# jorr3/Alphazero-4-player-chess

Measured on AMD Instinct MI355X. Metric: MCTS simulations/sec (whole node), 256 games×400 sims, 10-block ResNet, higher is better.
Workload: dtype fp16

## Files before the change

### alphazero-4-player-chess_amd/csrc/fpc_nn.h

```cpp
#pragma once
#include <hip/hip_runtime.h>

#include <algorithm>
#include <cstdlib>
#include <cstring>
#include <string>
#include <vector>

#include "fpc_tree_kernels.h"
#include "fpc_pack.h"
#include "fpc_tower.h"
#include "fpc_towerw.h"

namespace fpc {

typedef __attribute__((ext_vector_type(8))) __bf16 bf16x8_t;
typedef __attribute__((ext_vector_type(8))) _Float16 f16x8_t;
typedef __attribute__((ext_vector_type(16))) float f32x16_t;
typedef __attribute__((ext_vector_type(4))) uint32_t u32x4_t;
typedef __attribute__((ext_vector_type(2))) uint32_t u32x2_t;
typedef __attribute__((ext_vector_type(4))) float f32x4_t;

template <int DT>
struct E16;
// ... 334 lines not shown
  hipStream_t stream = nullptr;
  std::vector<void *> allocs;
  uint16_t *in16 = nullptr;
  uint16_t *act[3] = {nullptr, nullptr, nullptr};
  uint16_t *yv = nullptr;
  uint16_t *xfc = nullptr;
  float *d_logits = nullptr;
  float *d_stats = nullptr;
  float *d_value = nullptr;
  ConvW stem, pconv, vconv;
  std::vector<ConvW> c1, c2;
  uint16_t *fcw = nullptr;
  float *fcb = nullptr, *vw = nullptr;
  float *fc_part = nullptr;
  int fc_G1 = 0, fc_s1 = FC_SPLITK, fc_s2 = FC_SPLITK;
  int fc_layout = 1;
  int fc_gw = 256;
  unsigned char *towerW = nullptr;
  unsigned char *stemW = nullptr;
  float *towerB = nullptr;
  bool use_tower = false;
  int tower_waves = 8;
  bool tower_compact = true;
  bool tower_taploop = true;
  int towerw_rows = 1;
  bool use_towerw = false;
  void (*mark_fn)(void *, int) = nullptr;
  void *mark_ctx = nullptr;
  float vb = 0.f;
  bool attr_conv[2][3] = {{false, false, false}, {false, false, false}}, attr_tower[2] = {false, false}, attr_towerw[2] = {false, false}, attr_fc[2] = {false, false}, attr_gemv = false;

  template <class T>
  int dmalloc(T **p, size_t count, std::string *err) {
    void *q = nullptr;
    if (hipMalloc(&q, count * sizeof(T)) != hipSuccess) { *err = "hipMalloc failed in NN (" + std::to_string(count * sizeof(T)) + " bytes)"; return FPC_ENOMEM; }
    (void)hipMemset(q, 0, count * sizeof(T));
    allocs.push_back(q);
    *p = (T *)q;
    return 0;
  }

  int init(const DevCfg &c, int max_games, int nn_dtype, hipStream_t s, std::string *) {
    dc = c; Gmax = max_games; dtype = nn_dtype ? 1 : 0; stream = s;
    P = c.R + 2; PP = P * P;
    Mrows = ((max_games * PP + CONV_BM - 1) / CONV_BM) * CONV_BM;
    Gpad = ((max_games + 255) / 256) * 256;
// ... 77 lines not shown
    c1.assign(nblocks, ConvW()); c2.assign(nblocks, ConvW());
    for (int i = 0; i < nblocks; ++i) { if ((rc = conv(c1[i], F, Fp)) || (rc = conv(c2[i], F, Fp))) return rc; }
    if ((rc = conv(pconv, F, 128))) return rc;
    if ((rc = conv(vconv, F, 128))) return rc;
    if ((rc = dmalloc(&fcw, (size_t)Np * Kp, err)) || (rc = dmalloc(&fcb, (size_t)Np, err))) return rc;
    if ((rc = dmalloc(&vw, (size_t)dc.RR * 32, err))) return rc;
    const size_t rows = (size_t)Mrows + 2 * guard;
    if ((rc = dmalloc(&in16, rows * 32, err))) return rc;
    for (auto &a : act) if ((rc = dmalloc(&a, rows * F, err))) return rc;
    if ((rc = dmalloc(&yv, rows * 32, err))) return rc;
    if ((rc = dmalloc(&xfc, (size_t)Gpad * Kp, err))) return rc;
    if ((rc = dmalloc(&fc_part, (size_t)2 * FC_SPLITK * Gpad * Np, err))) return rc;
    plan_fc();
    if ((rc = dmalloc(&d_logits, (size_t)Gmax * dc.A, err))) return rc;
    if ((rc = dmalloc(&d_stats, (size_t)Gmax * SM_MAXCH * SM_REC, err))) return rc;
    if ((rc = dmalloc(&d_value, (size_t)Gmax, err))) return rc;
    use_tower = use_towerw = false;
    const bool dev = getenv("FPC_DEV_KNOBS") && atoi(getenv("FPC_DEV_KNOBS")) != 0;
    auto knob = [dev](const char *name, int dflt) { const char *v = dev ? getenv(name) : nullptr; return v ? atoi(v) : dflt; };
    const bool no_tower = knob("FPC_NO_TOWER", 0) != 0;
    tower_waves = knob("FPC_TOWER_WAVES", 8);
    tower_compact = knob("FPC_TOWER_COMPACT", 1) != 0;
    tower_taploop = knob("FPC_TOWER_TAPLOOP", 1) != 0;
    if (F == 256 && !no_tower) {
      use_towerw = true;
      towerw_rows = knob("FPC_TOWERW_ROWS", 1);
    } else if (F == 128 && !no_tower) {
      const int kw = knob("FPC_TOWERW", -1);
      use_towerw = kw < 0 ? dc.R != 14 : kw != 0;
      use_tower = !use_towerw;
    }
    const int layers = 2 * nblocks + 2;
    if (use_towerw) {
      const int slab = tww_slab(F), ksn = F / 32;
      if ((rc = dmalloc(&towerW, ((size_t)layers * 9 * ksn + TWW_PAD_SLABS) * slab, err)) || (rc = dmalloc(&stemW, (size_t)9 * slab, err)) ||
          (rc = dmalloc(&towerB, (size_t)layers * 256, err))) return rc;
    } else if (use_tower) {
      if ((rc = dmalloc(&towerW, (size_t)(layers * 9 + 3) * TW_TAP, err)) || (rc = dmalloc(&stemW, (size_t)9 * TW_STEM_TAP, err)) ||
          (rc = dmalloc(&towerB, (size_t)layers * 256, err))) return rc;
    }
    return 0;
  }
  std::vector<ConvW *> convs_in_blob_order() {
    std::vector<ConvW *> v{&stem};
    for (int i = 0; i < nblocks; ++i) { v.push_back(&c1[i]); v.push_back(&c2[i]); }
    v.push_back(&pconv); v.push_back(&vconv);
// ... 103 lines not shown
      in_boards = nullptr;
      t.in16 = in16 + (size_t)guard * 32; t.Wstem = stemW; t.bstem = stem.b; t.Wt = towerW; t.bt = towerB;
      t.xfc = xfc; t.vw = vw; t.value = value_out; t.vb = vb;
      t.L = 2 * nblocks; t.P = P; t.R = dc.R; t.PP = PP; t.NR = PP - P; t.T0 = (P + 1) / 16; t.n_games = n; t.Kp = Kp; t.A_ch = dc.A_ch; t.rules = dc.rules;
#if defined(TW_STAMPS) || defined(TWW_STAMPS)
      static unsigned long long *d_stamps = nullptr;
      if (!d_stamps) { (void)hipMalloc(&d_stamps, 2 * 8 * 16 * 8); }
      (void)hipMemsetAsync(d_stamps, 0, 2 * 8 * 16 * 8, stream);
      t.stamps = d_stamps;
#endif
      const int mt = dc.R <= 8 ? 3 : dc.R <= 11 ? 5 : 7;
      bool &attr = attr_tower[DT];
      if (!attr) {
        (void)hipFuncSetAttribute(reinterpret_cast<const void *>(&k_tower<DT, 3, false, 4>), hipFuncAttributeMaxDynamicSharedMemorySize, TW_LDS);
        (void)hipFuncSetAttribute(reinterpret_cast<const void *>(&k_tower<DT, 5, false, 4>), hipFuncAttributeMaxDynamicSharedMemorySize, TW_LDS);
        (void)hipFuncSetAttribute(reinterpret_cast<const void *>(&k_tower<DT, 7, false, 4>), hipFuncAttributeMaxDynamicSharedMemorySize, TW_LDS);
        (void)hipFuncSetAttribute(reinterpret_cast<const void *>(&k_tower<DT, 7, true, 4>), hipFuncAttributeMaxDynamicSharedMemorySize, TW_LDS);
        (void)hipFuncSetAttribute(reinterpret_cast<const void *>(&k_tower<DT, 7, true, 8>), hipFuncAttributeMaxDynamicSharedMemorySize, TW_LDS);
        (void)hipFuncSetAttribute(reinterpret_cast<const void *>(&k_tower<DT, 3, false, 8>), hipFuncAttributeMaxDynamicSharedMemorySize, TW_LDS);
        (void)hipFuncSetAttribute(reinterpret_cast<const void *>(&k_tower<DT, 5, false, 8>), hipFuncAttributeMaxDynamicSharedMemorySize, TW_LDS);
        (void)hipFuncSetAttribute(reinterpret_cast<const void *>(&k_tower<DT, 7, false, 8>), hipFuncAttributeMaxDynamicSharedMemorySize, TW_LDS);
        (void)hipFuncSetAttribute(reinterpret_cast<const void *>(&k_towerc<DT, false>), hipFuncAttributeMaxDynamicSharedMemorySize, TW_LDS);
        (void)hipFuncSetAttribute(reinterpret_cast<const void *>(&k_towerc<DT, true>), hipFuncAttributeMaxDynamicSharedMemorySize, TW_LDS);
        attr = true;
      }
      if (use_towerw) {
        bool &aw = attr_towerw[DT];
        if (!aw) {
#define FPC_TWW_ATTR(F_, MT_) (void)hipFuncSetAttribute(reinterpret_cast<const void *>(&k_towerw<DT, F_, MT_>), hipFuncAttributeMaxDynamicSharedMemorySize, tww_lds(F_))
#define FPC_TWW_ATTRS(F_) FPC_TWW_ATTR(F_, 2); FPC_TWW_ATTR(F_, 3); FPC_TWW_ATTR(F_, 4); FPC_TWW_ATTR(F_, 5); FPC_TWW_ATTR(F_, 6); FPC_TWW_ATTR(F_, 7)
          FPC_TWW_ATTRS(256); FPC_TWW_ATTRS(128);
#define FPC_TWW_ATTR1(F_, MT_) (void)hipFuncSetAttribute(reinterpret_cast<const void *>(&k_towerw<DT, F_, MT_, true>), hipFuncAttributeMaxDynamicSharedMemorySize, tww_lds(F_))
          FPC_TWW_ATTR1(128, 4); FPC_TWW_ATTR1(256, 4); FPC_TWW_ATTR1(256, 6); FPC_TWW_ATTR1(256, 7); FPC_TWW_ATTR1(256, 8);
          FPC_TWW_ATTR1(256, 9); FPC_TWW_ATTR1(256, 11); FPC_TWW_ATTR1(256, 13);
#undef FPC_TWW_ATTR1
          aw = true;
        }
        const int mtw = tww_mt(dc.R);
        if (mtw < 2 || mtw > 7) { *err = "k_towerw: board size outside 8..14"; return FPC_EINVAL; }
#define FPC_TWW_GO(F_, MT_) hipLaunchKernelGGL((k_towerw<DT, F_, MT_>), dim3(n), dim3(TWW_THREADS), tww_lds(F_), stream, t)
#define FPC_TWW_GOS(F_) switch (mtw) { case 2: FPC_TWW_GO(F_, 2); break; case 3: FPC_TWW_GO(F_, 3); break; case 4: FPC_TWW_GO(F_, 4); break; \
                                       case 5: FPC_TWW_GO(F_, 5); break; case 6: FPC_TWW_GO(F_, 6); break; default: FPC_TWW_GO(F_, 7); break; }
        const int tiles = tww_tiles(dc.R);
        const bool onerow = tiles <= 4 || (F == 256 && towerw_rows != 2);
#define FPC_TWW_GO1(F_, MT_) hipLaunchKernelGGL((k_towerw<DT, F_, MT_, true>), dim3(n), dim3(TWW_THREADS), tww_lds(F_), stream, t)
        if (onerow && F == 128) FPC_TWW_GO1(128, 4);
        else if (onerow) {
          switch (tiles) {
            case 4: FPC_TWW_GO1(256, 4); break;   case 6: FPC_TWW_GO1(256, 6); break;   case 7: FPC_TWW_GO1(256, 7); break;
            case 8: FPC_TWW_GO1(256, 8); break;   case 9: FPC_TWW_GO1(256, 9); break;   case 11: FPC_TWW_GO1(256, 11); break;
            default: FPC_TWW_GO1(256, 13); break;
          }
        } else if (F == 256) { FPC_TWW_GOS(256) } else { FPC_TWW_GOS(128) }
#undef FPC_TWW_GO1
#undef FPC_TWW_GOS
#undef FPC_TWW_GO
      } else if (mt == 3 && tower_waves == 8) hipLaunchKernelGGL((k_tower<DT, 3, false, 8>), dim3(n), dim3(512), TW_LDS, stream, t);
      else if (mt == 3) hipLaunchKernelGGL((k_tower<DT, 3, false, 4>), dim3(n), dim3(256), TW_LDS, stream, t);
      else if (mt == 5 && tower_waves == 8) hipLaunchKernelGGL((k_tower<DT, 5, false, 8>), dim3(n), dim3(512), TW_LDS, stream, t);
      else if (mt == 5) hipLaunchKernelGGL((k_tower<DT, 5, false, 4>), dim3(n), dim3(256), TW_LDS, stream, t);
      else if (P != 16 && tower_waves == 8) hipLaunchKernelGGL((k_tower<DT, 7, false, 8>), dim3(n), dim3(512), TW_LDS, stream, t);
      else if (P != 16) hipLaunchKernelGGL((k_tower<DT, 7, false, 4>), dim3(n), dim3(256), TW_LDS, stream, t);
      else if (tower_waves == 8 && tower_compact && dc.R == 14 && tower_taploop) hipLaunchKernelGGL((k_towerc<DT, true>), dim3(n), dim3(512), TW_LDS, stream, t);
      else if (tower_waves == 8 && tower_compact && dc.R == 14) hipLaunchKernelGGL((k_towerc<DT, false>), dim3(n), dim3(512), TW_LDS, stream, t);
      else if (tower_waves == 8) hipLaunchKernelGGL((k_tower<DT, 7, true, 8>), dim3(n), dim3(512), TW_LDS, stream, t);
      else hipLaunchKernelGGL((k_tower<DT, 7, true, 4>), dim3(n), dim3(256), TW_LDS, stream, t);
      const hipError_t le = hipGetLastError();
      if (le != hipSuccess) { *err = std::string("k_tower launch failed: ") + hipGetErrorString(le); return FPC_ENODEVICE; }
#if defined(TW_STAMPS) || defined(TWW_STAMPS)
      if (getenv("FPC_TW_STAMPS_FILE")) {
        unsigned long long h[2 * 8 * 16];
        (void)hipStreamSynchronize(stream);
        (void)hipMemcpy(h, t.stamps, sizeof(h), hipMemcpyDeviceToHost);
        if (FILE *f = fopen(getenv("FPC_TW_STAMPS_FILE"), "w")) {
          for (int i = 0; i < 2 * 8 * 16; ++i) fprintf(f, "%llu%c", h[i], i % 16 == 15 ? '\n' : ' ');
          fclose(f);
        }
      }
#endif
    } else if ((rc = conv(stem, in16, 32, nullptr, act[0], F, F, 0))) return rc;
    const bool fused = use_tower || use_towerw;
    for (int i = 0; i < nblocks && !fused; ++i) {
      const int t1 = (cur + 1) % 3, t2 = (cur + 2) % 3;
      if ((rc = conv(c1[i], act[cur], F, nullptr, act[t1], F, F, 0))) return rc;
      if ((rc = conv(c2[i], act[t1], F, act[cur], act[t2], F, F, 0))) return rc;
// ... 92 lines not shown
```

### alphazero-4-player-chess_amd/csrc/fpc_tower.h

```cpp
#pragma once
#include <hip/hip_runtime.h>

#include <type_traits>

#include "fpc_tree_kernels.h"

namespace fpc {

typedef __attribute__((ext_vector_type(8))) __bf16 t_bf16x8;
typedef __attribute__((ext_vector_type(8))) _Float16 t_f16x8;
typedef __attribute__((ext_vector_type(4))) float t_f32x4;
typedef __attribute__((ext_vector_type(2))) float t_f32x2;
typedef __attribute__((ext_vector_type(4))) uint32_t t_u32x4;
typedef __attribute__((ext_vector_type(2))) uint32_t t_u32x2;
typedef __attribute__((ext_vector_type(2))) short t_i16x2;

template <int DT>
struct M16;
template <>
struct M16<0> {
  static __device__ __forceinline__ t_f32x4 mfma(t_u32x4 a, t_u32x4 b, t_f32x4 c) {
    return __builtin_amdgcn_mfma_f32_16x16x32_bf16(__builtin_bit_cast(t_bf16x8, a), __builtin_bit_cast(t_bf16x8, b), c, 0, 0, 0);
  }
  static __device__ __forceinline__ uint32_t pack2(float lo, float hi) {
// ... 17 lines not shown
};
__device__ __forceinline__ uint32_t tw_relu2(uint32_t p) {
  return __builtin_bit_cast(uint32_t, __builtin_elementwise_max(__builtin_bit_cast(t_i16x2, p), (t_i16x2{0, 0})));
}

__host__ __device__ constexpr int tw_lay(int CH, int row, int c) {
  return (row >> 3) * (CH * 128) + (c >> 1) * 256 + (c & 1) * 128 + (row & 7) * 16;
}

constexpr int TW_THREADS = 256;
constexpr int TW_BIAS = 0;
constexpr int TW_DUMMY = 2048;
constexpr int TW_VRED = 2560;
constexpr int TW_BOARD = 2624;
constexpr int TW_PACE = 2944;
constexpr int TW_IMG0 = 4096;
constexpr int TW_IMG = 61440;
constexpr int TW_TAP = 32768;
constexpr int TW_RING = TW_IMG0 + TW_IMG;
constexpr int TW_LDS = TW_RING + 3 * TW_TAP;
constexpr int TW_STEM_TAP = 8192;
constexpr int TW_ENC = TW_RING + 9 * TW_STEM_TAP;
static_assert(TW_LDS == 163840, "k_tower uses the whole LDS of a CU");

struct TowerArgs {
  const fpc_board *boards;
  const int *leaf_slot, *leaf_turn;
  int board_stride;
  uint16_t one16;
  const uint16_t *in16;
  const unsigned char *Wstem;
  const float *bstem;
  const unsigned char *Wt;
  const float *bt;
  uint16_t *xfc;
  const float *vw;
  float *value;
  float vb;
  int L, P, R, PP, NR, T0, n_games, Kp, A_ch;
  int rules;
  unsigned long long *stamps;
};

__device__ __forceinline__ void tw_dma_8k(const unsigned char *gsrc_uniform, uint32_t lane_off, uint32_t lds_addr_uniform) {
  uint32_t keep;
  asm volatile(
      "s_mov_b32 %0, m0\n\ts_mov_b32 m0, %3\n\ts_nop 0\n\t"
      "global_load_lds_dwordx4 %1, %2\n\ts_add_u32 m0, m0, 0x400\n\tv_add_u32 %1, 0x400, %1\n\t"
      "global_load_lds_dwordx4 %1, %2\n\ts_add_u32 m0, m0, 0x400\n\tv_add_u32 %1, 0x400, %1\n\t"
      "global_load_lds_dwordx4 %1, %2\n\ts_add_u32 m0, m0, 0x400\n\tv_add_u32 %1, 0x400, %1\n\t"
      "global_load_lds_dwordx4 %1, %2\n\ts_add_u32 m0, m0, 0x400\n\tv_add_u32 %1, 0x400, %1\n\t"
      "global_load_lds_dwordx4 %1, %2\n\ts_add_u32 m0, m0, 0x400\n\tv_add_u32 %1, 0x400, %1\n\t"
      "global_load_lds_dwordx4 %1, %2\n\ts_add_u32 m0, m0, 0x400\n\tv_add_u32 %1, 0x400, %1\n\t"
      "global_load_lds_dwordx4 %1, %2\n\ts_add_u32 m0, m0, 0x400\n\tv_add_u32 %1, 0x400, %1\n\t"
      "global_load_lds_dwordx4 %1, %2\n\t"
      "s_mov_b32 m0, %0"
      : "=&s"(keep), "+v"(lane_off) : "s"(gsrc_uniform), "s"(lds_addr_uniform) : "memory", "scc");
}
__device__ __forceinline__ void tw_dma_4k(const unsigned char *gsrc_uniform, uint32_t lane_off, uint32_t lds_addr_uniform) {
  uint32_t keep;
  asm volatile(
      "s_mov_b32 %0, m0\n\ts_mov_b32 m0, %3\n\ts_nop 0\n\t"
      "global_load_lds_dwordx4 %1, %2\n\ts_add_u32 m0, m0, 0x400\n\tv_add_u32 %1, 0x400, %1\n\t"
      "global_load_lds_dwordx4 %1, %2\n\ts_add_u32 m0, m0, 0x400\n\tv_add_u32 %1, 0x400, %1\n\t"
      "global_load_lds_dwordx4 %1, %2\n\ts_add_u32 m0, m0, 0x400\n\tv_add_u32 %1, 0x400, %1\n\t"
      "global_load_lds_dwordx4 %1, %2\n\t"
      "s_mov_b32 m0, %0"
      : "=&s"(keep), "+v"(lane_off) : "s"(gsrc_uniform), "s"(lds_addr_uniform) : "memory", "scc");
}
template <int OFF>
__device__ __forceinline__ void tw_dma_piece(const unsigned char *gsrc_uniform, uint32_t lane_off) {
  asm volatile("global_load_lds_dwordx4 %0, %1 offset:%2" : : "v"(lane_off), "s"(gsrc_uniform), "i"(OFF) : "memory");
}
__device__ __forceinline__ void tw_set_m0(uint32_t lds_addr_uniform) {
  asm volatile("s_mov_b32 m0, %0\n\ts_nop 0" : : "s"(lds_addr_uniform) : "memory");
}
__device__ __forceinline__ void tw_dma_256(const unsigned char *gsrc_uniform, uint32_t lane_off, uint32_t lds_addr_uniform) {
  uint32_t keep;
  asm volatile("s_mov_b32 %0, m0\n\ts_mov_b32 m0, %3\n\ts_nop 0\n\tglobal_load_lds_dword %1, %2\n\ts_mov_b32 m0, %0"
               : "=&s"(keep) : "v"(lane_off), "s"(gsrc_uniform), "s"(lds_addr_uniform) : "memory");
}

#ifdef TW_STAMPS
#define TW_STAMP(GT, I)                                                                                       \
  do {                                                                                                        \
    if (g.stamps && blockIdx.x == 0 && ((GT) == TW_STAMPS || (GT) == TW_STAMPS + 1)) {                        \
      const unsigned long long t_ = __builtin_amdgcn_s_memtime();                                             \
// ... 3 lines not shown
#else
#define TW_STAMP(GT, I) do {} while (0)
#endif
#ifndef TW_AHEAD
#define TW_AHEAD 2
#endif
#ifndef TW_LOADERS
#define TW_LOADERS 1
#endif
#ifndef TW_STAGGER
#define TW_STAGGER 3
#endif
#ifndef TW_STRIP
#define TW_STRIP 0
#endif
#ifndef TWC_LOADER_TILES
#define TWC_LOADER_TILES 6
#endif

#ifndef TWC_STAGGER
#define TWC_STAGGER 2
#endif

template <int DT, int MT, bool FAST, int NW, int LOAD, bool CMP = false, bool TU = false>
__device__ __forceinline__ void tw_body(const TowerArgs &g) {
  static_assert(!CMP || (!FAST && NW == 8 && TW_LOADERS == 1 && MT == (LOAD == 2 ? TWC_LOADER_TILES : 13 - TWC_LOADER_TILES)), "compact form: 8 waves, 13 row tiles");
  static_assert(!TU || (CMP && TW_STAGGER != 0 && TWC_STAGGER >= 1 && TWC_STAGGER <= 3), "tap-specialised loop: compact form with the burst stream");
  constexpr int CR = 14, CZ = 16;
  constexpr int TB0 = LOAD == 2 ? 0 : TWC_LOADER_TILES;
  constexpr int NT = NW * 64;
  constexpr int WN = NW / 2;
  constexpr int CT = 8 / WN;
  constexpr int PIECES = 4 * LOAD;
  constexpr int DMA_PER_WAVE = PIECES * 1024;
  constexpr int MID = PIECES == 8 ? 4096 : 0;
  constexpr bool STREAM = TW_AHEAD == 2 && !(TW_STAGGER != 0 && NW == 8 && TW_LOADERS == 1);
  constexpr int STAG = (NW == 8 && TW_LOADERS == 1 && LOAD == 0) ? (TU ? TWC_STAGGER : TW_STAGGER) : 0;
  extern __shared__ __attribute__((aligned(16))) unsigned char smem[];
  unsigned char *const img = smem + TW_IMG0;
  unsigned char *const ring = smem + TW_RING;
  const float *const biasbuf = reinterpret_cast<const float *>(smem + TW_BIAS);
  float *const vred = reinterpret_cast<float *>(smem + TW_VRED);
  fpc_board *const lboard = reinterpret_cast<fpc_board *>(smem + TW_BOARD);
  const int tid = threadIdx.x, lane = tid & 63;
  const int wave = __builtin_amdgcn_readfirstlane(tid >> 6);
  const int wm = wave / WN, wn = wave % WN;
  const int li = lane & 15, lq = lane >> 4;
  const int game = blockIdx.x;
  const int P = g.P, NR = g.NR;

  int slot = 0, rot_k = 0;
  if (g.boards) {
    slot = g.leaf_slot[game];
    if (slot < 0) return;
    rot_k = first_leaf_turn(g.leaf_slot, g.leaf_turn, g.n_games);
  }

  const int rbase = CMP ? CZ + TB0 * 16 + li : (g.T0 + wm * MT) * 16 + li;
  uint32_t inmask = 0;
#pragma unroll
  for (int mt = 0; mt < MT; ++mt) {
    const int r = rbase + 16 * mt;
    if (CMP) {
      if (r - CZ < CR * CR) inmask |= 1u << mt;
    } else {
      const int pi = r / P, pj = r - pi * P;
      if (r < g.PP && pi >= 1 && pi <= g.R && pj >= 1 && pj <= g.R) inmask |= 1u << mt;
    }
  }
  auto colmask = [](int mt, int dx) -> uint64_t {
    uint32_t m16 = 0;
    for (int i = 0; i < 16; ++i)
      if (dx != 0 && ((TB0 + mt) * 16 + i) % CR == (dx < 0 ? 0 : CR - 1)) m16 |= 1u << i;
    const uint32_t m32 = m16 * 0x10001u;
    return ((uint64_t)m32 << 32) | m32;
  };
  auto lane_select = [](uint32_t a, uint32_t b, uint64_t m) -> uint32_t {
    uint32_t r;
    asm("v_cndmask_b32_e64 %0, %1, %2, %3" : "=v"(r) : "v"(a), "v"(b), "s"(m));
    return r;
  };
  const int bq = (lq >> 1) * 256 + (lq & 1) * 128;
  const int apart = (li >> 3) * 2048 + (li & 7) * 16 + bq;
  const int apart_s = (li >> 3) * 512 + (li & 7) * 16 + bq;
  const int cb64 = wn * (CT * 16);
  const int cb16 = (wn & 1) * 16;
  const bool vactive = wn < 2;

  for (int c = tid; c < (TW_IMG0 + TW_IMG) / 16; c += NT) reinterpret_cast<t_u32x4 *>(smem)[c] = t_u32x4{0u, 0u, 0u, 0u};
  unsigned char *const enc = smem + TW_ENC;
  const int enc_bytes = CMP ? 240 * 64 : ((NR + 7) >> 3) * 512;
  for (int c = tid; c < enc_bytes / 16; c += NT) reinterpret_cast<t_u32x4 *>(enc)[c] = t_u32x4{0u, 0u, 0u, 0u};
  {
    const t_u32x4 *src = reinterpret_cast<const t_u32x4 *>(g.Wstem);
    t_u32x4 *dst = reinterpret_cast<t_u32x4 *>(ring);
    for (int c = tid; c < 9 * TW_STEM_TAP / 16; c += NT) dst[c] = src[c];
  }
  t_f32x4 bst[CT];
#pragma unroll
  for (int ct = 0; ct < CT; ++ct) bst[ct] = *reinterpret_cast<const t_f32x4 *>(g.bstem + cb64 + ct * 16 + 4 * lq);
  __syncthreads();
  if (g.boards) {
    constexpr int WPB = (int)(sizeof(fpc_board) / 4);
    if (tid < WPB) reinterpret_cast<uint32_t *>(lboard)[tid] =
        reinterpret_cast<const uint32_t *>(g.boards + (size_t)game * g.board_stride + slot)[tid];
    __syncthreads();
    if (g.rules & FPC_RULES_ROTATION) rot_k = lboard->turn;
    for (int r = tid; r < (CMP ? CR * CR : g.PP); r += NT) {
      const int pi = CMP ? r / CR + 1 : r / P, pj = CMP ? r % CR + 1 : r - pi * P;
      if (pi < 1 || pi > g.R || pj < 1 || pj > g.R) continue;
      const uint8_t p = lboard->sq[rot90_src(g.R, rot_k, pi - 1, pj - 1)];
      if (!present(p)) continue;
      const int plane = piece_plane(p, lboard->turn, g.rules);
      *reinterpret_cast<uint16_t *>(enc + tw_lay(4, CMP ? CZ + r : r, plane >> 3) + (plane & 7) * 2) = g.one16;
    }
  } else if (CMP) {
    const uint16_t *src = g.in16 + (size_t)game * g.PP * 32;
    for (int c = tid; c < CR * CR * 4; c += NT) {
      const int q = c >> 2, j = c & 3;
      *reinterpret_cast<t_u32x4 *>(enc + tw_lay(4, CZ + q, j)) =
          *reinterpret_cast<const t_u32x4 *>(src + ((size_t)(q / CR + 1) * P + q % CR + 1) * 32 + j * 8);
    }
  } else {
    const uint16_t *src = g.in16 + (size_t)game * g.PP * 32;
    for (int c = tid; c < NR * 4; c += NT) {
      const int r = c >> 2, j = c & 3;
      *reinterpret_cast<t_u32x4 *>(enc + tw_lay(4, r, j)) = *reinterpret_cast<const t_u32x4 *>(src + (size_t)r * 32 + j * 8);
    }
  }
  __syncthreads();

  t_f32x4 acc[MT][CT];
  t_u32x2 res[MT][CT];

  auto brow = [&](int mt, int shift) -> int {
    int r = rbase + 16 * mt + shift;
    r = r < 0 ? r + NR : r;
    r = r >= NR ? r - NR : r;
    return r;
  };

#pragma unroll
  for (int tap = 0; tap < 9; ++tap) {
    const int shift = (tap / 3 - 1) * (CMP ? CR : P) + (tap % 3 - 1);
    t_u32x4 fa[CT], fb[MT];
#pragma unroll
    for (int ct = 0; ct < CT; ++ct)
      fa[ct] = *reinterpret_cast<const t_u32x4 *>(ring + tap * TW_STEM_TAP + (cb64 + ct * 16) * 64 + apart_s);
#pragma unroll
    for (int mt = 0; mt < MT; ++mt) {
      const int r = CMP ? (int)lane_select((uint32_t)(rbase + 16 * mt + shift), (uint32_t)((rbase + shift) & 7), colmask(mt, tap % 3 - 1)) : brow(mt, shift);
      fb[mt] = *reinterpret_cast<const t_u32x4 *>(enc + (r >> 3) * 512 + (r & 7) * 16 + bq);
    }
#pragma unroll
    for (int mt = 0; mt < MT; ++mt)
#pragma unroll
      for (int ct = 0; ct < CT; ++ct) acc[mt][ct] = M16<DT>::mfma(fa[ct], fb[mt], tap == 0 ? bst[ct] : acc[mt][ct]);
  }
  __syncthreads();

  const int total = (g.L + 2) * 9;
  const uint32_t dma_lane = (uint32_t)lane * 16u;
  const int lw = LOAD == 2 ? (wave & 3) : wave;
  auto issue_bias = [&](int T) {
    if (T % 9 == 0 && T < total && wave < 4) {
      const int l = T / 9;
      tw_dma_256(reinterpret_cast<const unsigned char *>(g.bt + (size_t)l * 256 + wave * 64), (uint32_t)lane * 4u,
                 (uint32_t)__builtin_amdgcn_readfirstlane(TW_BIAS + ((l & 1) * 256 + wave * 64) * 4));
    }
  };
  auto issue_tap = [&](int T) {
    issue_bias(T);
    if (LOAD == 0 || (TW_STRIP & 4)) return;
    const unsigned char *src = g.Wt + (size_t)T * TW_TAP + lw * DMA_PER_WAVE;
    const uint32_t dst = (uint32_t)__builtin_amdgcn_readfirstlane(TW_RING + (T % 3) * TW_TAP + lw * DMA_PER_WAVE);
    if (PIECES == 8) tw_dma_8k(src, dma_lane, dst);
    else tw_dma_4k(src, dma_lane, dst);
  };
  const unsigned char *dsrc = g.Wt;
  auto open_tap = [&](int T) {
    issue_bias(T);
    if (LOAD == 0) return;
    dsrc = g.Wt + (size_t)T * TW_TAP + lw * DMA_PER_WAVE + MID;
    tw_set_m0((uint32_t)__builtin_amdgcn_readfirstlane(TW_RING + (T % 3) * TW_TAP + lw * DMA_PER_WAVE + MID));
  };
  auto piece = [&](auto i_c) {
    constexpr int I = decltype(i_c)::value;
    if (LOAD != 0) tw_dma_piece<I * 1024 - MID>(dsrc, dma_lane);
  };
  issue_tap(0);
  issue_tap(1);
  if (STREAM) {
    open_tap(2);
    piece(std::integral_constant<int, 0>{});
    if (LOAD == 2) piece(std::integral_constant<int, 1>{});
  }

  unsigned char *const dummy = smem + TW_DUMMY + lane * 8;
  unsigned char *const wbase = img + (rbase >> 3) * 2048 + (rbase & 7) * 16 + wn * (CT * 256) + (lane >> 5) * 128 + ((lane >> 4) & 1) * 8;
  auto epilogue = [&](auto res_c) {
    constexpr int RES = decltype(res_c)::value;
    if (TW_STRIP & 16) return;
#pragma unroll
    for (int mt = 0; mt < MT; ++mt) {
      unsigned char *dst = ((inmask >> mt) & 1u) ? wbase + mt * 4096 : dummy;
#pragma unroll
      for (int ct = 0; ct < CT; ++ct) {
        t_f32x4 v = acc[mt][ct];
        if (RES == 2) {
          v[0] += M16<DT>::lo(res[mt][ct][0]); v[1] += M16<DT>::hi(res[mt][ct][0]);
          v[2] += M16<DT>::lo(res[mt][ct][1]); v[3] += M16<DT>::hi(res[mt][ct][1]);
        }
        const t_u32x2 pk = t_u32x2{tw_relu2(M16<DT>::pack2(v[0], v[1])), tw_relu2(M16<DT>::pack2(v[2], v[3]))};
        if (RES != 0) res[mt][ct] = pk;
        *reinterpret_cast<t_u32x2 *>(((inmask >> mt) & 1u) ? dst + ct * 256 : dst) = pk;
      }
      __builtin_amdgcn_sched_barrier(0);
    }
  };
  const std::integral_constant<int, 0> c0{};
  const std::integral_constant<int, 1> c1{};
  const std::integral_constant<int, 2> c2{};
  const std::integral_constant<int, 3> c3{};
  epilogue(c1);
  if (TW_STRIP & 32) { asm volatile("s_waitcnt vmcnt(0)" ::: "memory"); return; }
  if (STREAM) asm volatile("s_waitcnt vmcnt(%0)" ::"n"(PIECES + LOAD) : "memory");
  else asm volatile("s_waitcnt vmcnt(0)" ::: "memory");
  __syncthreads();

  t_u32x4 fa[2][CT], fb[2][MT];
  int gt = 0;
  const unsigned char *wslot;
  const unsigned char *bbase;
  const unsigned char *blast;
  int boff[FAST ? 1 : MT];
  auto set_tap = [&](int tap, int cb) {
    wslot = ring + (gt % 3) * TW_TAP + cb * 256 + apart;
    const int shift = (tap / 3 - 1) * P + (tap % 3 - 1);
    if (FAST) {
      const int r = rbase + shift;
      bbase = img + (r >> 3) * 2048 + (r & 7) * 16 + bq;
      int rl = r + 16 * (MT - 1);
      rl = rl >= NR ? rl - NR : rl;
      blast = img + (rl >> 3) * 2048 + (rl & 7) * 16 + bq;
    } else if (CMP) {
      const int dx = tap % 3 - 1;
      const int r = rbase + (tap / 3 - 1) * CR + dx;
      const uint32_t zoff = (r & 7) * 16 + bq;
      const uint32_t b0 = (r >> 3) * 2048 + zoff;
// ... 16 lines not shown
    asm volatile("" : "+v"(o2));
    wrow = ring + o;
    wrow2 = ring + o2;
  };
  int rrow = rbase - CR;
  auto set_tap_u = [&](auto xn_c) {
    constexpr int XN = decltype(xn_c)::value;
    wslot = XN == 2 ? wrow2 : wrow + XN * TW_TAP;
    const int r = rrow + (XN - 1);
    const uint32_t zoff = (r & 7) * 16 + bq;
    const uint32_t b0 = (r >> 3) * 2048 + zoff;
#pragma unroll
    for (int mt = 0; mt < MT; ++mt)
      boff[mt] = XN == 1 ? (int)(b0 + mt * 4096) : (int)lane_select(b0 + mt * 4096, zoff, colmask(mt, XN - 1));
  };
  auto bptr = [&](int mt) -> const unsigned char * {
    if (FAST) return mt == MT - 1 ? blast : bbase + mt * 4096;
    return img + boff[mt];
  };
  auto kstep = [&](auto mode_c, auto buf_c, auto ksn_c, auto bias_c, const t_f32x4 *b4, auto q_c) {
    constexpr int MODE = decltype(mode_c)::value, B = decltype(buf_c)::value, KSN = decltype(ksn_c)::value;
    constexpr bool BIAS = decltype(bias_c)::value != 0;
    constexpr int N = B ^ 1, Q = decltype(q_c)::value;
    if (!(TW_STRIP & 2)) {
#pragma unroll
      for (int ct = 0; ct < CT; ++ct) fa[N][ct] = *reinterpret_cast<const t_u32x4 *>(wslot + ct * 4096 + KSN * 512);
      fb[N][0] = *reinterpret_cast<const t_u32x4 *>(bptr(0) + KSN * 512);
    }
    __builtin_amdgcn_sched_barrier(0);
#pragma unroll
    for (int mt = 0; mt < MT; ++mt) {
      if (TW_STRIP & 1) {
        if (BIAS) {
#pragma unroll
          for (int ct = 0; ct < (MODE == 0 ? CT : 1); ++ct) acc[mt][ct] = b4[ct];
        }
        asm volatile("" : "+v"(fa[B][0]), "+v"(fb[B][mt]));
      } else if (MODE == 0) {
#pragma unroll
        for (int ct = 0; ct < CT; ++ct) acc[mt][ct] = M16<DT>::mfma(fa[B][ct], fb[B][mt], BIAS ? b4[ct] : acc[mt][ct]);
      } else if (NW == 4 || vactive) {
        acc[mt][0] = M16<DT>::mfma(fa[B][0], fb[B][mt], BIAS ? b4[0] : acc[mt][0]);
      }
      __builtin_amdgcn_sched_barrier(0);
      if (mt + 1 < MT && !(TW_STRIP & 2)) {
        fb[N][mt + 1] = *reinterpret_cast<const t_u32x4 *>(bptr(mt + 1) + KSN * 512);
        __builtin_amdgcn_sched_barrier(0);
      }
      if (STREAM && LOAD != 0) {
        if (mt == (LOAD == 2 ? MT / 3 : MT / 2)) piece(std::integral_constant<int, LOAD * Q>{});
        if (LOAD == 2 && mt == (2 * MT) / 3) piece(std::integral_constant<int, LOAD * Q + 1>{});
        __builtin_amdgcn_sched_barrier(0);
      }
    }
  };
  auto load_b0 = [&]() {
#pragma unroll
    for (int mt = 0; mt < MT; ++mt) fb[0][mt] = *reinterpret_cast<const t_u32x4 *>(bptr(mt));
  };
  const unsigned char *usrc = g.Wt + (size_t)TW_TAP + lw * DMA_PER_WAVE;
  const uint32_t udst = (uint32_t)__builtin_amdgcn_readfirstlane(TW_RING + lw * DMA_PER_WAVE);
  auto tap_u = [&](auto mode_c, auto x_c, const t_f32x4 *b4, const int dy, const int cb_next) {
    constexpr int X = decltype(x_c)::value;
    if (STAG == 2) {
      TW_STAMP(gt, 3);
      __syncthreads();
      TW_STAMP(gt, 4);
    }
    TW_STAMP(gt, 0);
    kstep(mode_c, c1, c2, c0, b4, c2);
    TW_STAMP(gt, 1);
    if (STAG == 1) __syncthreads();
    kstep(mode_c, c0, c3, c0, b4, c3);
    TW_STAMP(gt, 2);
    if (!STAG) {
      asm volatile("s_waitcnt vmcnt(0)" ::: "memory");
      TW_STAMP(gt, 3);
      if (!(TW_STRIP & 8)) __syncthreads();
      TW_STAMP(gt, 4);
      if (LOAD != 0 && !(TW_STRIP & 4)) {
        usrc += TW_TAP;
        tw_dma_8k(usrc, dma_lane, udst + ((X + 2) % 3) * TW_TAP);
      }
      TW_STAMP(gt, 5);
    }
    ++gt;
    if (X == 2) {
      rrow = dy == 1 ? rbase - CR : rrow + CR;
      if (dy == 1) set_wrow(cb_next);
    }
    set_tap_u(std::integral_constant<int, (X + 1) % 3>{});
    TW_STAMP(gt - 1, 6);
    kstep(mode_c, c1, c0, c0, b4, c0);
    TW_STAMP(gt - 1, 7);
  };
  auto run_layer = [&](auto mode_c, const int layer, const int cb, const int cb_next) {
    constexpr int MODE = decltype(mode_c)::value;
    if (TU && wave < 4 && layer + 1 < g.L + 2)
      tw_dma_256(reinterpret_cast<const unsigned char *>(g.bt + (size_t)(layer + 1) * 256 + wave * 64), (uint32_t)lane * 4u,
                 (uint32_t)__builtin_amdgcn_readfirstlane(TW_BIAS + (((layer + 1) & 1) * 256 + wave * 64) * 4));
    t_f32x4 b4[CT];
    {
      const float *bl = biasbuf + (layer & 1) * 256 + cb + 4 * lq;
#pragma unroll
      for (int ct = 0; ct < (MODE == 0 ? CT : 1); ++ct) b4[ct] = *reinterpret_cast<const t_f32x4 *>(bl + ct * 16);
// ... 57 lines not shown
  if (TU) {
    set_wrow(cb64);
    set_tap_u(c0);
  } else {
    set_tap(0, cb64);
  }
#pragma unroll
  for (int ct = 0; ct < CT; ++ct) fa[0][ct] = *reinterpret_cast<const t_u32x4 *>(wslot + ct * 4096);
  load_b0();
  const int nblocks = g.L / 2;
#pragma unroll 1
  for (int blk = 0; blk < nblocks; ++blk) {
    run_layer(c0, 2 * blk, cb64, cb64);
    epilogue(c0);
    __syncthreads();
    load_b0();
    run_layer(c0, 2 * blk + 1, cb64, blk + 1 == nblocks ? cb16 : cb64);
    epilogue(c2);
    __syncthreads();
    load_b0();
  }
  float vpart = 0.f;
  {
    run_layer(c1, g.L, cb16, cb64);
#pragma unroll
    for (int mt = 0; mt < MT; ++mt) {
      const int r = rbase + 16 * mt;
      const int pi = r / P, pj = r - pi * P;
      const bool in = ((inmask >> mt) & 1u) && (NW == 4 || vactive);
      const int qp = !in ? 0 : CMP ? r - CZ : (pi - 1) * g.R + (pj - 1);
      const t_f32x4 w4 = *reinterpret_cast<const t_f32x4 *>(g.vw + qp * 32 + cb16 + 4 * lq);
#pragma unroll
      for (int j = 0; j < 4; ++j) {
        float v = acc[mt][0][j];
        v = v > 0.f ? v : 0.f;
        vpart += in ? v * w4[j] : 0.f;
      }
    }
  }
  run_layer(c0, g.L + 1, cb64, cb64);
  epilogue(c0);
  __syncthreads();

  if (!(TW_STRIP & 64)) {
    const int cpr = g.A_ch / 8;
    for (int c = tid; c < (CMP ? CR * CR : g.PP) * 16; c += NT) {
      const int j = c & 15;
// ... 6 lines not shown
        q = (pi - 1) * g.R + (pj - 1);
      }
      *reinterpret_cast<t_u32x4 *>(g.xfc + (size_t)game * g.Kp + (size_t)q * g.A_ch + j * 8) =
          *reinterpret_cast<const t_u32x4 *>(img + tw_lay(16, r, j));
    }
  }
  for (int off = 32; off >= 1; off >>= 1) vpart += __shfl_xor(vpart, off);
  if (lane == 0) vred[wave] = vpart;
  __syncthreads();
  if (tid == 0) g.value[game] = tanhf(g.vb + ((vred[0] + vred[1]) + (vred[WN] + vred[WN + 1])));
  asm volatile("s_waitcnt vmcnt(0)" ::: "memory");
}

template <int DT, int MT, bool FAST, int NW>
__global__ void __launch_bounds__(NW * 64, NW / 4) k_tower(TowerArgs g) {
  if (NW == 8 && TW_LOADERS == 1) {
    if (__builtin_amdgcn_readfirstlane(threadIdx.x >> 6) < 4) tw_body<DT, MT, FAST, NW, 2>(g);
    else tw_body<DT, MT, FAST, NW, 0>(g);
  } else {
    tw_body<DT, MT, FAST, NW, NW == 4 ? 2 : 1>(g);
  }
}

template <int DT, bool TU>
__global__ void __launch_bounds__(512, 2) k_towerc(TowerArgs g) {
  if (__builtin_amdgcn_readfirstlane(threadIdx.x >> 6) < 4) tw_body<DT, TWC_LOADER_TILES, false, 8, 2, true, TU>(g);
  else tw_body<DT, 13 - TWC_LOADER_TILES, false, 8, 0, true, TU>(g);
}

__global__ void __launch_bounds__(256) k_tower_prep(const uint16_t *W, unsigned char *out, int taps, int cin) {
  const int CH = cin / 8;
  const long c = (long)blockIdx.x * 256 + threadIdx.x;
  if (c >= (long)taps * 128 * CH) return;
  const int tap = (int)(c / (128 * CH)), rem = (int)(c % (128 * CH)), row = rem / CH, j = rem % CH;
  *reinterpret_cast<t_u32x4 *>(out + (size_t)tap * 128 * cin * 2 + tw_lay(CH, row, j)) =
      *reinterpret_cast<const t_u32x4 *>(W + ((size_t)tap * 128 + row) * cin + j * 8);
}

}
```

Before: 497,200.

## Add trimmed compact tower variant with async stem load and slimmer value-head stream

Adds a TRIM specialisation of the compact tap-loop tower kernel, which becomes the default for 14x14 boards. The stem weights move from a cooperative LDS copy to async global-to-LDS DMA into free ring and image regions. Only the image border rows are zeroed, and the board fetch and first-leaf ballot overlap with those loads. During the value-head layer it streams only the needed 2KB slice per tap, and inactive waves skip its MFMAs. The complex LDS aliasing and vmcnt accounting risk correctness and hazard bugs.

```diff
diff --git a/alphazero-4-player-chess_amd/csrc/fpc_nn.h b/alphazero-4-player-chess_amd/csrc/fpc_nn.h
--- a/alphazero-4-player-chess_amd/csrc/fpc_nn.h
+++ b/alphazero-4-player-chess_amd/csrc/fpc_nn.h
@@ -380,6 +380,7 @@
   bool use_tower = false;
   int tower_waves = 8;
   bool tower_compact = true;
+  bool tower_trim = true;
   bool tower_taploop = true;
   int towerw_rows = 1;
   bool use_towerw = false;
@@ -503,6 +504,7 @@
     tower_waves = knob("FPC_TOWER_WAVES", 8);
     tower_compact = knob("FPC_TOWER_COMPACT", 1) != 0;
     tower_taploop = knob("FPC_TOWER_TAPLOOP", 1) != 0;
+    tower_trim = knob("FPC_TOWER_TRIM", 1) != 0;
     if (F == 256 && !no_tower) {
       use_towerw = true;
       towerw_rows = knob("FPC_TOWERW_ROWS", 1);
@@ -652,6 +654,7 @@
         (void)hipFuncSetAttribute(reinterpret_cast<const void *>(&k_tower<DT, 7, false, 8>), hipFuncAttributeMaxDynamicSharedMemorySize, TW_LDS);
         (void)hipFuncSetAttribute(reinterpret_cast<const void *>(&k_towerc<DT, false>), hipFuncAttributeMaxDynamicSharedMemorySize, TW_LDS);
         (void)hipFuncSetAttribute(reinterpret_cast<const void *>(&k_towerc<DT, true>), hipFuncAttributeMaxDynamicSharedMemorySize, TW_LDS);
+        (void)hipFuncSetAttribute(reinterpret_cast<const void *>(&k_towerc<DT, true, true>), hipFuncAttributeMaxDynamicSharedMemorySize, TW_LDS);
         attr = true;
       }
       if (use_towerw) {
@@ -691,6 +694,7 @@
       else if (mt == 5) hipLaunchKernelGGL((k_tower<DT, 5, false, 4>), dim3(n), dim3(256), TW_LDS, stream, t);
       else if (P != 16 && tower_waves == 8) hipLaunchKernelGGL((k_tower<DT, 7, false, 8>), dim3(n), dim3(512), TW_LDS, stream, t);
       else if (P != 16) hipLaunchKernelGGL((k_tower<DT, 7, false, 4>), dim3(n), dim3(256), TW_LDS, stream, t);
+      else if (tower_waves == 8 && tower_compact && dc.R == 14 && tower_taploop && tower_trim) hipLaunchKernelGGL((k_towerc<DT, true, true>), dim3(n), dim3(512), TW_LDS, stream, t);
       else if (tower_waves == 8 && tower_compact && dc.R == 14 && tower_taploop) hipLaunchKernelGGL((k_towerc<DT, true>), dim3(n), dim3(512), TW_LDS, stream, t);
       else if (tower_waves == 8 && tower_compact && dc.R == 14) hipLaunchKernelGGL((k_towerc<DT, false>), dim3(n), dim3(512), TW_LDS, stream, t);
       else if (tower_waves == 8) hipLaunchKernelGGL((k_tower<DT, 7, true, 8>), dim3(n), dim3(512), TW_LDS, stream, t);
diff --git a/alphazero-4-player-chess_amd/csrc/fpc_tower.h b/alphazero-4-player-chess_amd/csrc/fpc_tower.h
--- a/alphazero-4-player-chess_amd/csrc/fpc_tower.h
+++ b/alphazero-4-player-chess_amd/csrc/fpc_tower.h
@@ -63,6 +63,16 @@
 constexpr int TW_STEM_TAP = 8192;
 constexpr int TW_ENC = TW_RING + 9 * TW_STEM_TAP;
 static_assert(TW_LDS == 163840, "k_tower uses the whole LDS of a CU");
+constexpr int TW_ENC_BYTES = 240 * 64;
+constexpr int TW_STEM_LO = TW_RING + TW_TAP;
+constexpr int TW_ENC_T = TW_STEM_LO + 5 * TW_STEM_TAP;
+constexpr int TW_STEM_HI = TW_IMG0 + 16 * 256;
+constexpr int TW_ZERO_HI = TW_IMG0 + 208 * 256;
+static_assert(TW_STEM_LO >= TW_RING + TW_TAP, "ring slot 0 stays free for residual tap 0");
+static_assert(TW_ENC_T + TW_ENC_BYTES <= TW_LDS, "stem taps 0..4 and the input image fit ring slots 1 and 2");
+static_assert(TW_STEM_HI + 4 * TW_STEM_TAP <= TW_ZERO_HI && TW_ZERO_HI <= TW_IMG0 + (16 + 196) * 256,
+              "stem taps 5..8 lie in rows of squares, clear of the rows that are zeroed");
+static_assert(TW_ZERO_HI % 2048 == 0 && (TW_IMG0 + TW_IMG - TW_ZERO_HI) % 16 == 0, "whole 8-row groups are cleared");
 
 struct TowerArgs {
   const fpc_board *boards;
@@ -104,6 +114,20 @@
       "s_mov_b32 %0, m0\n\ts_mov_b32 m0, %3\n\ts_nop 0\n\t"
       "global_load_lds_dwordx4 %1, %2\n\ts_add_u32 m0, m0, 0x400\n\tv_add_u32 %1, 0x400, %1\n\t"
       "global_load_lds_dwordx4 %1, %2\n\ts_add_u32 m0, m0, 0x400\n\tv_add_u32 %1, 0x400, %1\n\t"
+      "global_load_lds_dwordx4 %1, %2\n\ts_add_u32 m0, m0, 0x400\n\tv_add_u32 %1, 0x400, %1\n\t"
+      "global_load_lds_dwordx4 %1, %2\n\t"
+      "s_mov_b32 m0, %0"
+      : "=&s"(keep), "+v"(lane_off) : "s"(gsrc_uniform), "s"(lds_addr_uniform) : "memory", "scc");
+}
+__device__ __forceinline__ void tw_dma_1k(const unsigned char *gsrc_uniform, uint32_t lane_off, uint32_t lds_addr_uniform) {
+  uint32_t keep;
+  asm volatile("s_mov_b32 %0, m0\n\ts_mov_b32 m0, %3\n\ts_nop 0\n\tglobal_load_lds_dwordx4 %1, %2\n\ts_mov_b32 m0, %0"
+               : "=&s"(keep) : "v"(lane_off), "s"(gsrc_uniform), "s"(lds_addr_uniform) : "memory");
+}
+__device__ __forceinline__ void tw_dma_2k(const unsigned char *gsrc_uniform, uint32_t lane_off, uint32_t lds_addr_uniform) {
+  uint32_t keep;
+  asm volatile(
+      "s_mov_b32 %0, m0\n\ts_mov_b32 m0, %3\n\ts_nop 0\n\t"
       "global_load_lds_dwordx4 %1, %2\n\ts_add_u32 m0, m0, 0x400\n\tv_add_u32 %1, 0x400, %1\n\t"
       "global_load_lds_dwordx4 %1, %2\n\t"
       "s_mov_b32 m0, %0"
@@ -153,8 +177,9 @@
 #define TWC_STAGGER 2
 #endif
 
-template <int DT, int MT, bool FAST, int NW, int LOAD, bool CMP = false, bool TU = false>
+template <int DT, int MT, bool FAST, int NW, int LOAD, bool CMP = false, bool TU = false, bool TRIM = false>
 __device__ __forceinline__ void tw_body(const TowerArgs &g) {
+  static_assert(!TRIM || TU, "the trimmed head / value stream / tail belong to the tap-specialised loop");
   static_assert(!CMP || (!FAST && NW == 8 && TW_LOADERS == 1 && MT == (LOAD == 2 ? TWC_LOADER_TILES : 13 - TWC_LOADER_TILES)), "compact form: 8 waves, 13 row tiles");
   static_assert(!TU || (CMP && TW_STAGGER != 0 && TWC_STAGGER >= 1 && TWC_STAGGER <= 3), "tap-specialised loop: compact form with the burst stream");
   constexpr int CR = 14, CZ = 16;
@@ -180,8 +205,46 @@
   const int game = blockIdx.x;
   const int P = g.P, NR = g.NR;
 
+  const int total = (g.L + 2) * 9;
+  const uint32_t dma_lane = (uint32_t)lane * 16u;
+  const int lw = LOAD == 2 ? (wave & 3) : wave;
+  auto issue_bias = [&](int T) {
+    if (T % 9 == 0 && T < total && wave < 4) {
+      const int l = T / 9;
+      tw_dma_256(reinterpret_cast<const unsigned char *>(g.bt + (size_t)l * 256 + wave * 64), (uint32_t)lane * 4u,
+                 (uint32_t)__builtin_amdgcn_readfirstlane(TW_BIAS + ((l & 1) * 256 + wave * 64) * 4));
+    }
+  };
+  auto issue_tap = [&](int T) {
+    issue_bias(T);
+    if (LOAD == 0 || (TW_STRIP & 4)) return;
+    const unsigned char *src = g.Wt + (size_t)T * TW_TAP + lw * DMA_PER_WAVE;
+    const uint32_t dst = (uint32_t)__builtin_amdgcn_readfirstlane(TW_RING + (T % 3) * TW_TAP + lw * DMA_PER_WAVE);
+    if (PIECES == 8) tw_dma_8k(src, dma_lane, dst);
+    else tw_dma_4k(src, dma_lane, dst);
+  };
+
   int slot = 0, rot_k = 0;
-  if (g.boards) {
+  int ls64 = -1, lt64 = 0;
+  t_f32x4 bst[CT];
+  if (TRIM) {
+    if (g.boards) {
+      const int g64 = lane < g.n_games ? lane : g.n_games - 1;
+      ls64 = g.leaf_slot[g64];
+      lt64 = g.leaf_turn[g64];
+    }
+#pragma unroll
+    for (int ct = 0; ct < CT; ++ct) bst[ct] = *reinterpret_cast<const t_f32x4 *>(g.bstem + wn * (CT * 16) + ct * 16 + 4 * lq);
+    tw_dma_4k(g.Wstem + wave * 5120, dma_lane, (uint32_t)__builtin_amdgcn_readfirstlane(TW_STEM_LO + wave * 5120));
+    tw_dma_1k(g.Wstem + wave * 5120 + 4096, dma_lane, (uint32_t)__builtin_amdgcn_readfirstlane(TW_STEM_LO + wave * 5120 + 4096));
+    tw_dma_4k(g.Wstem + 5 * TW_STEM_TAP + wave * 4096, dma_lane, (uint32_t)__builtin_amdgcn_readfirstlane(TW_STEM_HI + wave * 4096));
+    if (g.boards)
+      asm volatile("s_load_dword %0, %1, 0x0\n\ts_waitcnt lgkmcnt(0)" : "=s"(slot) : "s"(g.leaf_slot + game) : "memory");
+    if (slot < 0) {
+      asm volatile("s_waitcnt vmcnt(0)" ::: "memory");
+      return;
+    }
+  } else if (g.boards) {
     slot = g.leaf_slot[game];
     if (slot < 0) return;
     rot_k = first_leaf_turn(g.leaf_slot, g.leaf_turn, g.n_games);
@@ -218,24 +281,40 @@
   const int cb16 = (wn & 1) * 16;
   const bool vactive = wn < 2;
 
-  for (int c = tid; c < (TW_IMG0 + TW_IMG) / 16; c += NT) reinterpret_cast<t_u32x4 *>(smem)[c] = t_u32x4{0u, 0u, 0u, 0u};
-  unsigned char *const enc = smem + TW_ENC;
-  const int enc_bytes = CMP ? 240 * 64 : ((NR + 7) >> 3) * 512;
-  for (int c = tid; c < enc_bytes / 16; c += NT) reinterpret_cast<t_u32x4 *>(enc)[c] = t_u32x4{0u, 0u, 0u, 0u};
-  {
-    const t_u32x4 *src = reinterpret_cast<const t_u32x4 *>(g.Wstem);
-    t_u32x4 *dst = reinterpret_cast<t_u32x4 *>(ring);
-    for (int c = tid; c < 9 * TW_STEM_TAP / 16; c += NT) dst[c] = src[c];
-  }
-  t_f32x4 bst[CT];
-#pragma unroll
-  for (int ct = 0; ct < CT; ++ct) bst[ct] = *reinterpret_cast<const t_f32x4 *>(g.bstem + cb64 + ct * 16 + 4 * lq);
+  constexpr int WPB = (int)(sizeof(fpc_board) / 4);
+  unsigned char *const enc = smem + (TRIM ? TW_ENC_T : TW_ENC);
+  const int enc_bytes = CMP ? TW_ENC_BYTES : ((NR + 7) >> 3) * 512;
+  if (TRIM) {
+    uint32_t bword = 0;
+    if (g.boards && tid < WPB) bword = reinterpret_cast<const uint32_t *>(g.boards + (size_t)game * g.board_stride + slot)[tid];
+    for (int c = tid; c < 16 * 256 / 16; c += NT) reinterpret_cast<t_u32x4 *>(smem + TW_IMG0)[c] = t_u32x4{0u, 0u, 0u, 0u};
+    for (int c = tid; c < (TW_IMG0 + TW_IMG - TW_ZERO_HI) / 16; c += NT) reinterpret_cast<t_u32x4 *>(smem + TW_ZERO_HI)[c] = t_u32x4{0u, 0u, 0u, 0u};
+    for (int c = tid; c < enc_bytes / 16; c += NT) reinterpret_cast<t_u32x4 *>(enc)[c] = t_u32x4{0u, 0u, 0u, 0u};
+    if (g.boards) {
+      asm volatile("" : "+v"(ls64), "+v"(lt64));
+      const unsigned long long bal = __ballot(lane < g.n_games && ls64 >= 0);
+      rot_k = bal ? wave_read(lt64, (int)__ffsll((long long)bal) - 1)
+                  : g.n_games > 64 ? first_leaf_turn(g.leaf_slot, g.leaf_turn, g.n_games) : 0;
+      if (tid < WPB) reinterpret_cast<uint32_t *>(lboard)[tid] = bword;
+    }
+  } else {
+    for (int c = tid; c < (TW_IMG0 + TW_IMG) / 16; c += NT) reinterpret_cast<t_u32x4 *>(smem)[c] = t_u32x4{0u, 0u, 0u, 0u};
+    for (int c = tid; c < enc_bytes / 16; c += NT) reinterpret_cast<t_u32x4 *>(enc)[c] = t_u32x4{0u, 0u, 0u, 0u};
+    {
+      const t_u32x4 *src = reinterpret_cast<const t_u32x4 *>(g.Wstem);
+      t_u32x4 *dst = reinterpret_cast<t_u32x4 *>(ring);
+      for (int c = tid; c < 9 * TW_STEM_TAP / 16; c += NT) dst[c] = src[c];
+    }
+#pragma unroll
+    for (int ct = 0; ct < CT; ++ct) bst[ct] = *reinterpret_cast<const t_f32x4 *>(g.bstem + cb64 + ct * 16 + 4 * lq);
+  }
   __syncthreads();
   if (g.boards) {
-    constexpr int WPB = (int)(sizeof(fpc_board) / 4);
-    if (tid < WPB) reinterpret_cast<uint32_t *>(lboard)[tid] =
-        reinterpret_cast<const uint32_t *>(g.boards + (size_t)game * g.board_stride + slot)[tid];
-    __syncthreads();
+    if (!TRIM) {
+      if (tid < WPB) reinterpret_cast<uint32_t *>(lboard)[tid] =
+          reinterpret_cast<const uint32_t *>(g.boards + (size_t)game * g.board_stride + slot)[tid];
+      __syncthreads();
+    }
     if (g.rules & FPC_RULES_ROTATION) rot_k = lboard->turn;
     for (int r = tid; r < (CMP ? CR * CR : g.PP); r += NT) {
       const int pi = CMP ? r / CR + 1 : r / P, pj = CMP ? r % CR + 1 : r - pi * P;
@@ -259,6 +338,12 @@
       *reinterpret_cast<t_u32x4 *>(enc + tw_lay(4, r, j)) = *reinterpret_cast<const t_u32x4 *>(src + (size_t)r * 32 + j * 8);
     }
   }
+  if (TRIM) {
+    constexpr int TAP0 = LOAD == 2 ? ((TW_STRIP & 4) ? 1 : PIECES + 1) : 0;
+    static_assert(!TRIM || (NW == 8 && TW_LOADERS == 1), "the waves that carry tap 0 are the waves that carry the biases");
+    issue_tap(0);
+    asm volatile("s_waitcnt vmcnt(%0)" ::"n"(TAP0) : "memory");
+  }
   __syncthreads();
 
   t_f32x4 acc[MT][CT];
@@ -277,7 +362,8 @@
     t_u32x4 fa[CT], fb[MT];
 #pragma unroll
     for (int ct = 0; ct < CT; ++ct)
-      fa[ct] = *reinterpret_cast<const t_u32x4 *>(ring + tap * TW_STEM_TAP + (cb64 + ct * 16) * 64 + apart_s);
+      fa[ct] = *reinterpret_cast<const t_u32x4 *>((!TRIM ? ring + tap * TW_STEM_TAP : tap < 5 ? smem + TW_STEM_LO + tap * TW_STEM_TAP : smem + TW_STEM_HI + (tap - 5) * TW_STEM_TAP) +
+                                                  (cb64 + ct * 16) * 64 + apart_s);
 #pragma unroll
     for (int mt = 0; mt < MT; ++mt) {
       const int r = CMP ? (int)lane_select((uint32_t)(rbase + 16 * mt + shift), (uint32_t)((rbase + shift) & 7), colmask(mt, tap % 3 - 1)) : brow(mt, shift);
@@ -290,24 +376,6 @@
   }
   __syncthreads();
 
-  const int total = (g.L + 2) * 9;
-  const uint32_t dma_lane = (uint32_t)lane * 16u;
-  const int lw = LOAD == 2 ? (wave & 3) : wave;
-  auto issue_bias = [&](int T) {
-    if (T % 9 == 0 && T < total && wave < 4) {
-      const int l = T / 9;
-      tw_dma_256(reinterpret_cast<const unsigned char *>(g.bt + (size_t)l * 256 + wave * 64), (uint32_t)lane * 4u,
-                 (uint32_t)__builtin_amdgcn_readfirstlane(TW_BIAS + ((l & 1) * 256 + wave * 64) * 4));
-    }
-  };
-  auto issue_tap = [&](int T) {
-    issue_bias(T);
-    if (LOAD == 0 || (TW_STRIP & 4)) return;
-    const unsigned char *src = g.Wt + (size_t)T * TW_TAP + lw * DMA_PER_WAVE;
-    const uint32_t dst = (uint32_t)__builtin_amdgcn_readfirstlane(TW_RING + (T % 3) * TW_TAP + lw * DMA_PER_WAVE);
-    if (PIECES == 8) tw_dma_8k(src, dma_lane, dst);
-    else tw_dma_4k(src, dma_lane, dst);
-  };
   const unsigned char *dsrc = g.Wt;
   auto open_tap = [&](int T) {
     issue_bias(T);
@@ -319,7 +387,7 @@
     constexpr int I = decltype(i_c)::value;
     if (LOAD != 0) tw_dma_piece<I * 1024 - MID>(dsrc, dma_lane);
   };
-  issue_tap(0);
+  if (!TRIM) issue_tap(0);
   issue_tap(1);
   if (STREAM) {
     open_tap(2);
@@ -356,6 +424,7 @@
   epilogue(c1);
   if (TW_STRIP & 32) { asm volatile("s_waitcnt vmcnt(0)" ::: "memory"); return; }
   if (STREAM) asm volatile("s_waitcnt vmcnt(%0)" ::"n"(PIECES + LOAD) : "memory");
+  else if (TRIM) asm volatile("s_waitcnt vmcnt(%0)" ::"n"(LOAD != 0 && !(TW_STRIP & 4) ? PIECES : 0) : "memory");
   else asm volatile("s_waitcnt vmcnt(0)" ::: "memory");
   __syncthreads();
 
@@ -418,9 +487,11 @@
     constexpr int MODE = decltype(mode_c)::value, B = decltype(buf_c)::value, KSN = decltype(ksn_c)::value;
     constexpr bool BIAS = decltype(bias_c)::value != 0;
     constexpr int N = B ^ 1, Q = decltype(q_c)::value;
+    constexpr bool VQ = TRIM && MODE == 1;
+    if (MODE == 2) return;
     if (!(TW_STRIP & 2)) {
 #pragma unroll
-      for (int ct = 0; ct < CT; ++ct) fa[N][ct] = *reinterpret_cast<const t_u32x4 *>(wslot + ct * 4096 + KSN * 512);
+      for (int ct = 0; ct < (VQ ? 1 : CT); ++ct) fa[N][ct] = *reinterpret_cast<const t_u32x4 *>(wslot + ct * 4096 + KSN * 512);
       fb[N][0] = *reinterpret_cast<const t_u32x4 *>(bptr(0) + KSN * 512);
     }
     __builtin_amdgcn_sched_barrier(0);
@@ -435,7 +506,7 @@
       } else if (MODE == 0) {
 #pragma unroll
         for (int ct = 0; ct < CT; ++ct) acc[mt][ct] = M16<DT>::mfma(fa[B][ct], fb[B][mt], BIAS ? b4[ct] : acc[mt][ct]);
-      } else if (NW == 4 || vactive) {
+      } else if (VQ || NW == 4 || vactive) {
         acc[mt][0] = M16<DT>::mfma(fa[B][0], fb[B][mt], BIAS ? b4[0] : acc[mt][0]);
       }
       __builtin_amdgcn_sched_barrier(0);
@@ -456,6 +527,9 @@
   };
   const unsigned char *usrc = g.Wt + (size_t)TW_TAP + lw * DMA_PER_WAVE;
   const uint32_t udst = (uint32_t)__builtin_amdgcn_readfirstlane(TW_RING + lw * DMA_PER_WAVE);
+  auto sgpr = [](uint32_t v) { return (uint32_t)__builtin_amdgcn_readfirstlane(v); };
+  const int vtap0 = 9 * g.L;
+  const uint32_t vback = (uint32_t)__builtin_amdgcn_readfirstlane(lw * (DMA_PER_WAVE - 2048));
   auto tap_u = [&](auto mode_c, auto x_c, const t_f32x4 *b4, const int dy, const int cb_next) {
     constexpr int X = decltype(x_c)::value;
     if (STAG == 2) {
@@ -476,7 +550,14 @@
       TW_STAMP(gt, 4);
       if (LOAD != 0 && !(TW_STRIP & 4)) {
         usrc += TW_TAP;
-        tw_dma_8k(usrc, dma_lane, udst + ((X + 2) % 3) * TW_TAP);
+        const int T = gt + 2;
+        if (!TRIM) {
+          tw_dma_8k(usrc, dma_lane, udst + ((X + 2) % 3) * TW_TAP);
+        } else if (T >= vtap0 && T < vtap0 + 9) {
+          tw_dma_2k(usrc - vback, dma_lane, sgpr(udst - vback + ((X + 2) % 3) * TW_TAP));
+        } else if (T < total) {
+          tw_dma_8k(usrc, dma_lane, sgpr(udst + ((X + 2) % 3) * TW_TAP));
+        }
       }
       TW_STAMP(gt, 5);
     }
@@ -580,7 +661,13 @@
   }
   float vpart = 0.f;
   {
-    run_layer(c1, g.L, cb16, cb64);
+    if (!TRIM || vactive) run_layer(c1, g.L, cb16, cb64);
+    else run_layer(c2, g.L, cb16, cb64);
+    if (TRIM) {
+#pragma unroll
+      for (int ct = 0; ct < CT; ++ct) fa[0][ct] = *reinterpret_cast<const t_u32x4 *>(wslot + ct * 4096);
+      load_b0();
+    }
 #pragma unroll
     for (int mt = 0; mt < MT; ++mt) {
       const int r = rbase + 16 * mt;
@@ -633,10 +720,10 @@
   }
 }
 
-template <int DT, bool TU>
+template <int DT, bool TU, bool TRIM = false>
 __global__ void __launch_bounds__(512, 2) k_towerc(TowerArgs g) {
-  if (__builtin_amdgcn_readfirstlane(threadIdx.x >> 6) < 4) tw_body<DT, TWC_LOADER_TILES, false, 8, 2, true, TU>(g);
-  else tw_body<DT, 13 - TWC_LOADER_TILES, false, 8, 0, true, TU>(g);
+  if (__builtin_amdgcn_readfirstlane(threadIdx.x >> 6) < 4) tw_body<DT, TWC_LOADER_TILES, false, 8, 2, true, TU, TRIM>(g);
+  else tw_body<DT, 13 - TWC_LOADER_TILES, false, 8, 0, true, TU, TRIM>(g);
 }
 
 __global__ void __launch_bounds__(256) k_tower_prep(const uint16_t *W, unsigned char *out, int taps, int cin) {
```

Result: no change. 498,900 (median of 6 runs) (+0.3%).
